# apache/bifromq

Measured on NVIDIA H100. Metric: publish-topics matched/sec @10M filters, higher is better.
Workload: dtype u8/u32 (byte and integer work)

## Files before the change

bifromq_b200/csrc/capi.cu:

```cuda
#include <cuda_runtime.h>

#include <algorithm>
#include <atomic>
#include <chrono>
#include <cstdio>
#include <cstdlib>
#include <cstring>
#include <memory>
#include <mutex>
#include <thread>
#include <string>
#include <vector>

#include "../../include/bfq_gpumatch.h"
#include "codec.h"
#include "cuda_buf.h"
#include "index_builder.h"
#include "fanout.h"
#include "lease.h"
#include "match_kernels.cuh"

using namespace bfq;

struct Snapshot {
    int device = 0;
    uint64_t generation = 0;
    DeviceBuf<Slot> d_slots, d_roots;
    DeviceBuf<uint32_t> d_segs, d_pfxP, d_pfxG;
    DeviceBuf<uint8_t> d_rkind, d_tags;
    FlatIndex flat;
    struct TenantHost {
        std::shared_ptr<const KVBlob> kv;
        std::shared_ptr<const std::vector<uint8_t>> rkind;
        std::shared_ptr<const TenantFan> fan;
    };
    struct FanTable {
        DeviceBuf<uint32_t> d_rdeliv, d_gmem_off, d_gmem_deliv;
        DeviceBuf<uint8_t> d_gordered;
        uint32_t n_deliverers = 0;
    };
    struct UrlTable {
        DeviceBuf<unsigned long long> d_words;
        DeviceBuf<long long> d_word;
        DeviceBuf<uint32_t> d_len;
        uint32_t member_bits = 1;
    };
    std::mutex fan_mu;
    std::shared_ptr<FanTable> fan;
    std::shared_ptr<UrlTable> urls;
    std::vector<TenantHost> th;
    uint64_t garbage_slots = 0;
    int64_t delta_commits = 0;
    size_t l2_window_bytes = 0;
    bool locate(int64_t rank, size_t* ti, int64_t* local) const {
        if (rank < 0 || rank >= flat.n_routes || flat.tenants.empty()) return false;
        size_t lo = 0, hi = flat.tenants.size();
        while (hi - lo > 1) {
            const size_t mid = (lo + hi) / 2;
            if (flat.tenants[mid].lo <= rank) lo = mid;
            else hi = mid;
        }
        *ti = lo;
        *local = rank - flat.tenants[lo].lo;
        return *local < flat.tenants[lo].n_routes;
    }
    int64_t device_bytes() const {
        return (int64_t) (d_slots.bytes() + d_tags.bytes() + d_roots.bytes() + d_segs.bytes() + d_rkind.bytes() + d_pfxP.bytes() + d_pfxG.bytes());
    }
    ~Snapshot() { cudaSetDevice(device); }
};

constexpr int MAX_CHUNKS = 8;

struct Workspace {
    int device = 0;
    cudaStream_t stream = nullptr, copy_stream = nullptr, work_stream[2] = {nullptr, nullptr};
    cudaEvent_t ev[2] = {nullptr, nullptr};
    cudaEvent_t ev_h2d[MAX_CHUNKS] = {};
    cudaEvent_t evk[2] = {nullptr, nullptr};
    cudaEvent_t ev_done = nullptr;
    std::vector<cudaEvent_t> ev_use;
    uint64_t tab_generation = ~0ull;
    std::vector<uint8_t> tab_blob;
    std::vector<int64_t> tab_off;
    std::vector<int32_t> tab_caps;
    int32_t tab_n = -1;
    bool any_cap = true;
    DeviceBuf<int32_t> d_tenant_tab;
    PinnedBuf<int32_t> h_tenant_tab;
    DeviceBuf<uint8_t> d_topics;
    DeviceBuf<int64_t> d_topic_off;
    DeviceBuf<int32_t> d_topic_tenant;
    DeviceBuf<uint32_t> d_span_begin, d_span_count, d_route_count, d_overflow, d_flagged, d_kept, d_defer;
    DeviceBuf<uint2> d_ranges, d_scratch, d_ranges_c;
    DeviceBuf<uint8_t> d_scan_tmp;
    DeviceBuf<uint32_t> d_cnt, d_new_begin, d_final_begin, d_final_count;
    DeviceBuf<uint32_t> d_ord_keys, d_leader, d_order;
    DeviceBuf<unsigned long long> d_hash_tab;
    DeviceBuf<uint32_t> d_hist;
    size_t hash_stride = 0, hist_stride = 0;
    DeviceBuf<uint3> d_throttled;
    DeviceBuf<unsigned long long> d_counters;
    PinnedBuf<unsigned long long> h_counters;
    DeviceBuf<unsigned long long> d_exp_counts;
    DeviceBuf<long long> d_bud_bytes;
    DeviceBuf<uint8_t> d_bud_bw, d_bud_flags;
    DeviceBuf<uint32_t> d_bud_dp, d_bud_list;
    DeviceBuf<unsigned long long> d_bud_ctr;
    DeviceBuf<uint32_t> d_fo_counts, d_fo_base, d_pack_topic, d_pack_rank, d_pack_member;
    DeviceBuf<long long> d_pack_offsets;
    DeviceBuf<uint8_t> d_fo_tmp;
    DeviceBuf<uint32_t> d_dl_topic_tmp, d_dl_pair_tmp, d_dl_pcount, d_package_tenant, d_dl_pack_topic, d_match_rank, d_match_member;
    DeviceBuf<unsigned long long> d_dl_totals;
    DeviceBuf<long long> d_package_off, d_dl_pack_off, d_match_off;
    DeviceBuf<uint8_t> d_dl_tmp;
    DeviceBuf<uint32_t> d_os_flag, d_os_u32, d_pack_pub;
    DeviceBuf<unsigned long long> d_os_items, d_os_check, d_os_key;
    DeviceBuf<long long> d_pack_pub_off;
    PinnedBuf<uint32_t> h_span_begin, h_span_count, h_route_count;
    PinnedBuf<uint2> h_ranges;
    PinnedBuf<uint3> h_throttled;

    cudaError_t init(int dev) {
        device = dev;
        cudaError_t e = cudaStreamCreateWithFlags(&stream, cudaStreamNonBlocking);
        if (e == cudaSuccess) e = cudaStreamCreateWithFlags(&copy_stream, cudaStreamNonBlocking);
        for (auto& w : work_stream)
            if (e == cudaSuccess) e = cudaStreamCreateWithFlags(&w, cudaStreamNonBlocking);
        for (auto& x : ev)
            if (e == cudaSuccess) e = cudaEventCreate(&x);
        for (auto& x : evk)
            if (e == cudaSuccess) e = cudaEventCreate(&x);
        for (auto& x : ev_h2d)
            if (e == cudaSuccess) e = cudaEventCreateWithFlags(&x, cudaEventDisableTiming);
        if (e == cudaSuccess) e = cudaEventCreateWithFlags(&ev_done, cudaEventDisableTiming);
        return e;
    }
    ~Workspace() {
        cudaSetDevice(device);
        for (auto& e : ev) if (e) cudaEventDestroy(e);
        for (auto& e : evk) if (e) cudaEventDestroy(e);
        for (auto& e : ev_h2d) if (e) cudaEventDestroy(e);
        if (ev_done) cudaEventDestroy(ev_done);
        for (auto& e : ev_use) cudaEventDestroy(e);
        if (copy_stream) cudaStreamDestroy(copy_stream);
        for (auto& w : work_stream) if (w) cudaStreamDestroy(w);
        if (stream) cudaStreamDestroy(stream);
    }
};

struct Pool {
    std::mutex mu;
    std::vector<Workspace*> idle;
    int device = 0;
    bool closed = false;
    ~Pool() {
        cudaSetDevice(device);
        for (Workspace* w : idle) delete w;
    }
};

struct bfq_result {
    bfq_index* owner = nullptr;
    std::shared_ptr<Pool> pool;
    std::shared_ptr<Snapshot> snap;
    Workspace* ws = nullptr;
    int64_t n_topics = 0, n_ranges = 0, n_throttled = 0;
    const uint32_t *span_begin = nullptr, *span_count = nullptr, *route_count = nullptr;
    const bfq_range* ranges = nullptr;
    const bfq_throttled* throttled = nullptr;
    double ms[4] = {0, 0, 0, 0};
};

struct bfq_index {
    int device = 0;
    std::mutex mu;
    std::mutex stage_mu;
    Staging staging;
    std::shared_ptr<Snapshot> snap;
    uint64_t next_generation = 1;
// ... 62 lines not shown
            pool->idle.push_back(w);
            return;
        }
    }
    cudaSetDevice(pool->device);
    delete w;
}

struct CoreOut {
    int64_t n_ranges = 0, n_throttled = 0, n_overflow = 0, n_flagged = 0, n_launches = 0, n_deferred = 0, n_leaders = 0;
    uint64_t want_dyn = 0, want_thr = 0;
    int64_t chunk_throttled[MAX_CHUNKS] = {};
};

int32_t resolve_tenants(Workspace* w, const Snapshot* s, const uint8_t* tenants, const int64_t* tenant_off, int32_t n_tenants,
                        const int32_t* max_p, const int32_t* max_g, cudaStream_t stream) {
    if (n_tenants < 0) return fail(BFQ_E_INVALID, "n_tenants < 0");
    if (n_tenants >= (1 << 30)) return fail(BFQ_E_RANGE, "more than 2^30 tenants in one batch");
    const size_t nt = (size_t) std::max(n_tenants, 1);
    const size_t blob_n = n_tenants ? (size_t) (tenant_off[n_tenants] - tenant_off[0]) : 0;
    bool same = w->tab_generation == s->generation && w->tab_n == n_tenants && w->tab_blob.size() == blob_n;
    if (same && n_tenants > 0) {
        same = memcmp(w->tab_blob.data(), tenants + tenant_off[0], blob_n) == 0;
        for (int32_t i = 0; same && i <= n_tenants; i++) same = w->tab_off[i] == tenant_off[i] - tenant_off[0];
        for (int32_t i = 0; same && i < n_tenants; i++)
            same = w->tab_caps[i] == (max_p ? max_p[i] : 0x7FFFFFFF) && w->tab_caps[nt + i] == (max_g ? max_g[i] : 0x7FFFFFFF);
    }
    if (same) return BFQ_OK;
    BFQ_CUDA_TRY(w->h_tenant_tab.reserve(3 * nt));
    BFQ_CUDA_TRY(w->d_tenant_tab.reserve(3 * nt));
    w->tab_blob.assign(tenants ? tenants + (n_tenants ? tenant_off[0] : 0) : nullptr, tenants ? tenants + (n_tenants ? tenant_off[0] : 0) + blob_n : nullptr);
    w->tab_off.resize(nt + 1);
    w->tab_caps.assign(2 * nt, 0x7FFFFFFF);
    bool any_cap = false;
    for (int32_t i = 0; i < n_tenants; i++) {
        std::string t((const char*) tenants + tenant_off[i], (size_t) (tenant_off[i + 1] - tenant_off[i]));
        auto it = s->flat.tenant_ordinal.find(t);
        const int32_t mp = max_p ? max_p[i] : 0x7FFFFFFF, mg = max_g ? max_g[i] : 0x7FFFFFFF;
        w->h_tenant_tab.p[i] = it == s->flat.tenant_ordinal.end() ? -1 : (int32_t) it->second;
        w->h_tenant_tab.p[nt + i] = mp;
        w->h_tenant_tab.p[2 * nt + i] = mg;
        w->tab_off[i] = tenant_off[i] - tenant_off[0];
        w->tab_caps[i] = mp;
        w->tab_caps[nt + i] = mg;
        any_cap = any_cap || mp != 0x7FFFFFFF || mg != 0x7FFFFFFF;
    }
    if (n_tenants > 0) w->tab_off[n_tenants] = tenant_off[n_tenants] - tenant_off[0];
    BFQ_CUDA_TRY(cudaMemcpyAsync(w->d_tenant_tab.p, w->h_tenant_tab.p, 3 * nt * sizeof(int32_t), cudaMemcpyHostToDevice, stream));
    w->tab_generation = s->generation;
    w->tab_n = n_tenants;
    w->any_cap = any_cap;
    return BFQ_OK;
}

struct SubBatch {
    int64_t begin = 0, n = 0, n_total = 0;
    int chunk = 0;
    uint64_t dyn_off = 0, dyn_cap = 0;
    uint64_t thr_off = 0, thr_cap = 0;
};
constexpr int32_t BFQ_RETRY_GROW = -100;

int32_t prepare_workspace(bfq_index* h, Workspace* w, int64_t n, int n_chunks, int32_t n_tenants) {
    const size_t nn = (size_t) std::max<int64_t>(n, 1);
    if (n >= (int64_t) 0x3FFFFFFF) return fail(BFQ_E_INVALID, "too many topics in one batch");
    BFQ_CUDA_TRY(w->d_span_begin.reserve(nn));
    BFQ_CUDA_TRY(w->d_span_count.reserve(nn));
    BFQ_CUDA_TRY(w->d_route_count.reserve(nn));
    BFQ_CUDA_TRY(w->d_overflow.reserve(nn));
    BFQ_CUDA_TRY(w->d_flagged.reserve(nn));
    BFQ_CUDA_TRY(w->d_kept.reserve(nn));
    BFQ_CUDA_TRY(w->d_defer.reserve(nn));
    BFQ_CUDA_TRY(w->d_counters.reserve(CTR_COUNT * MAX_CHUNKS));
    BFQ_CUDA_TRY(w->h_counters.reserve(CTR_COUNT * MAX_CHUNKS));
    const uint64_t dyn_base = (uint64_t) n * INLINE_RANGES;
    if (dyn_base >= 0xF0000000ull) return fail(BFQ_E_RANGE, "batch too large for 32-bit range indices; split the batch");
    const size_t min_dyn = std::max<size_t>((size_t) n_chunks << 18, nn);
    if (w->d_ranges.cap < dyn_base + min_dyn) BFQ_CUDA_TRY(w->d_ranges.reserve((size_t) (dyn_base + std::max<size_t>(1 << 20, min_dyn))));
    const int64_t per_chunk = (n + n_chunks - 1) / n_chunks + 1;
    if (per_chunk >= h->order_min) {
        BFQ_CUDA_TRY(w->d_ord_keys.reserve(nn));
        BFQ_CUDA_TRY(w->d_leader.reserve(nn));
        BFQ_CUDA_TRY(w->d_order.reserve(nn));
        const size_t hist_stride = order_scratch_words(per_chunk, n_tenants);
        const size_t hash_stride = order_hash_entries(per_chunk);
        if (hist_stride > w->hist_stride) {
            BFQ_CUDA_TRY(w->d_hist.reserve(2 * hist_stride));
            w->hist_stride = hist_stride;
        }
        if (hash_stride > w->hash_stride) {
            BFQ_CUDA_TRY(w->d_hash_tab.reserve(2 * hash_stride));
            w->hash_stride = hash_stride;
        }
    }
    if (w->d_throttled.cap < ((size_t) n_chunks << 14)) BFQ_CUDA_TRY(w->d_throttled.reserve(std::max<size_t>(1 << 16, (size_t) n_chunks << 14)));
    return BFQ_OK;
}

SubBatch whole_batch(Workspace* w, int64_t n) {
    SubBatch sb;
    sb.begin = 0;
    sb.n = sb.n_total = n;
    sb.dyn_cap = w->d_ranges.cap - (uint64_t) n * INLINE_RANGES;
    sb.thr_cap = w->d_throttled.cap;
    return sb;
}

struct CoreCtx {
    bfq_index* h;
    Workspace* w;
    const Snapshot* s;
    const uint8_t* d_topics;
    const int64_t* d_topic_off;
    const int32_t* d_topic_tenant;
    int32_t n_tenants;
    cudaStream_t stream;
};

MatchParams core_params(const CoreCtx& c, const SubBatch& sb) {
    Workspace* w = c.w;
    const size_t nt = (size_t) std::max(c.n_tenants, 1);
    const int64_t b = sb.begin;
    MatchParams p{};
    p.slots = c.s->d_slots.p;
    p.roots = c.s->d_roots.p;
    p.tags = reinterpret_cast<const uint4*>(c.s->d_tags.p);
    p.n_blocks = c.s->flat.n_blocks;
    p.topics = c.d_topics;
    p.topic_off = c.d_topic_off + b;
    p.topic_tenant = c.d_topic_tenant + b;
    p.tenant_root = w->d_tenant_tab.p;
    p.max_pfanout = w->d_tenant_tab.p + nt;
    p.max_gfanout = w->d_tenant_tab.p + 2 * nt;
    p.n_tenants = c.n_tenants;
    p.n_topics = sb.n;
    p.span_begin = w->d_span_begin.p + b;
    p.span_count = w->d_span_count.p + b;
    p.route_count = w->d_route_count.p + b;
    p.overflow_list = w->d_overflow.p + b;
    p.defer_list = w->d_defer.p + b;
    p.flagged_list = w->d_flagged.p + b;
    p.counters = w->d_counters.p + (size_t) sb.chunk * CTR_COUNT;
    p.ranges = w->d_ranges.p + (uint64_t) b * INLINE_RANGES;
    p.dyn_base = (uint64_t) (sb.n_total - b) * INLINE_RANGES + sb.dyn_off;
    p.ranges_cap = p.dyn_base + sb.dyn_cap;
    p.max_ctas_per_sm = c.h->tier0_ctas_per_sm;
    return p;
}

CapsParams caps_params(const CoreCtx& c, const SubBatch& sb, const MatchParams& p) {
    CapsParams q{};
    q.flagged_list = p.flagged_list;
    q.topic_tenant = p.topic_tenant;
    q.max_pfanout = p.max_pfanout;
    q.max_gfanout = p.max_gfanout;
    q.span_begin = p.span_begin;
    q.span_count = p.span_count;
    q.ranges = p.ranges;
    q.segs = c.s->d_segs.p;
    q.rkind = c.s->d_rkind.p;
    q.pfx_persistent = c.s->d_pfxP.p;
    q.pfx_group = c.s->d_pfxG.p;
    q.kept_count = c.w->d_kept.p + sb.begin;
    q.counters = p.counters;
    q.throttled = c.w->d_throttled.p + sb.thr_off;
    q.throttled_cap = sb.thr_cap;
    q.topic_base = (uint32_t) sb.begin;
    return q;
}

bool wants_order(const CoreCtx& c, const SubBatch& sb) {
    return sb.n >= c.h->order_min && c.w->d_order.cap >= (size_t) (sb.begin + sb.n) && c.w->hist_stride > 0 &&
           c.w->hist_stride >= order_scratch_words(sb.n, c.n_tenants) && c.w->hash_stride >= order_hash_entries(sb.n);
}

int32_t enqueue_core(const CoreCtx& c, const SubBatch& sb, CoreOut* out) {
    Workspace* w = c.w;
    cudaStream_t stream = c.stream;
    const int64_t n = sb.n, b = sb.begin;
    MatchParams p = core_params(c, sb);
    if (c.s->l2_window_bytes > 0) {
        cudaStreamAttrValue attr{};
        attr.accessPolicyWindow.base_ptr = c.s->d_tags.p;
        attr.accessPolicyWindow.num_bytes = c.s->l2_window_bytes;
        attr.accessPolicyWindow.hitRatio = 1.0f;
        attr.accessPolicyWindow.hitProp = cudaAccessPropertyPersisting;
        attr.accessPolicyWindow.missProp = cudaAccessPropertyStreaming;
        cudaStreamSetAttribute(stream, cudaStreamAttributeAccessPolicyWindow, &attr);
        cudaGetLastError();
    }
    BFQ_CUDA_TRY(cudaMemsetAsync(p.counters, 0, CTR_COUNT * sizeof(unsigned long long), stream));
    bool ordered = false, dedup = false;
    if (wants_order(c, sb)) {
        const int slot = sb.chunk & 1;
        OrderParams q{};
        q.n_topics = n;
        q.topics = c.d_topics;
        q.topic_off = p.topic_off;
        q.topic_tenant = p.topic_tenant;
        q.n_tenants = c.n_tenants;
        q.keys = w->d_ord_keys.p + b;
        q.leader = w->d_leader.p + b;
        q.order = w->d_order.p + b;
        q.hash_tab = w->d_hash_tab.p + (size_t) slot * w->hash_stride;
        q.hash_mask = order_hash_entries(n) - 1;
        q.hist = w->d_hist.p + (size_t) slot * w->hist_stride;
        q.dedup = c.h->dedup ? 1 : 0;
        q.dedup_hash_mask = c.h->dedup_hash_bits >= 64 ? ~0ull : (1ull << c.h->dedup_hash_bits) - 1;
        q.counters = p.counters;
        BFQ_CUDA_TRY(launch_order(q, stream));
        p.order = q.order;
        p.order_count = p.counters + CTR_NLEAD;
        out->n_launches += 3;
        ordered = true;
        dedup = q.dedup != 0;
    }
    if (n > 0) {
        if (sb.chunk == 0) BFQ_CUDA_TRY(cudaEventRecord(w->evk[0], stream));
        launch_match_lanes(p, stream);
        if (sb.chunk == 0) BFQ_CUDA_TRY(cudaEventRecord(w->evk[1], stream));
        p.work_list = p.defer_list;
        p.n_work = -1;
        launch_match(p, false, 0, stream);
        out->n_launches += 2;
        if (ordered && dedup) {
            FinalizeParams f{};
            f.n_topics = n;
            f.leader = w->d_leader.p + b;
            f.span_begin = p.span_begin;
            f.span_count = p.span_count;
            f.route_count = p.route_count;
            f.flagged_list = p.flagged_list;
            f.counters = p.counters;
            f.second_pass = 0;
            launch_finalize(f, stream);
            out->n_launches += 1;
        }
        if (w->any_cap) {
            CapsParams q = caps_params(c, sb, p);
            q.n_flagged = -1;
            launch_caps(q, stream);
            out->n_launches += 2;
        }
    }
    BFQ_CUDA_TRY(cudaGetLastError());
    return BFQ_OK;
}

int32_t copy_counters(const CoreCtx& c, const SubBatch& sb) {
    BFQ_CUDA_TRY(cudaMemcpyAsync(c.w->h_counters.p + (size_t) sb.chunk * CTR_COUNT, c.w->d_counters.p + (size_t) sb.chunk * CTR_COUNT,
                             CTR_COUNT * sizeof(unsigned long long), cudaMemcpyDeviceToHost, c.stream));
    return BFQ_OK;
}

int32_t finish_core(const CoreCtx& c, const SubBatch& sb, CoreOut* out, bool* reran, cudaEvent_t done = nullptr) {
    Workspace* w = c.w;
    cudaStream_t stream = c.stream;
    unsigned long long* hc = w->h_counters.p + (size_t) sb.chunk * CTR_COUNT;
    if (reran) *reran = false;
    if (done) BFQ_CUDA_TRY(cudaEventSynchronize(done));
    else BFQ_CUDA_TRY(cudaStreamSynchronize(stream));
    out->n_overflow += (int64_t) hc[CTR_OVERFLOW];
    out->n_deferred += (int64_t) hc[CTR_DEFER];
    if (hc[CTR_OVERFLOW] > 0) {
        MatchParams p = core_params(c, sb);
        const uint64_t capF = (uint64_t) c.s->flat.max_nodes_per_depth + 2;
        const uint64_t capR = 2 * ((uint64_t) c.s->flat.max_tenant_nodes + 2) + 2;
        const uint64_t per_warp = 4 * capF + capR;
        uint64_t warps = std::min<uint64_t>(hc[CTR_OVERFLOW], std::max<uint64_t>(8, (1ull << 31) / (per_warp * sizeof(uint2))));
        warps = std::min<uint64_t>(warps, (uint64_t) device_sm_count() * 8);
        warps = (warps + 7) / 8 * 8;
        if (w->d_scratch.cap < (size_t) (warps * per_warp)) {
            BFQ_CUDA_TRY(cudaDeviceSynchronize());
            BFQ_CUDA_TRY(w->d_scratch.reserve((size_t) (warps * per_warp)));
        }
        p.scratch = w->d_scratch.p;
        p.scratch_frontier_cap = capF;
        p.scratch_ranges_cap = capR;
        p.work_list = p.overflow_list;
        p.n_work = (int64_t) hc[CTR_OVERFLOW];
        launch_match(p, true, (int) warps, stream);
        out->n_launches++;
        if (w->hist_stride > 0 && c.h->dedup && wants_order(c, sb)) {
            FinalizeParams f{};
            f.n_topics = sb.n;
            f.leader = w->d_leader.p + sb.begin;
            f.span_begin = p.span_begin;
            f.span_count = p.span_count;
            f.route_count = p.route_count;
            f.flagged_list = p.flagged_list;
            f.counters = p.counters;
            f.second_pass = 1;
            launch_finalize(f, stream);
            out->n_launches++;
        }
        if (w->any_cap) {
            CapsParams q = caps_params(c, sb, p);
            q.n_flagged = -1;
            launch_caps(q, stream);
            out->n_launches += 2;
        }
        BFQ_CUDA_TRY(cudaGetLastError());
        int32_t rc = copy_counters(c, sb);
        if (rc != BFQ_OK) return rc;
        BFQ_CUDA_TRY(cudaStreamSynchronize(stream));
        if (hc[CTR_ERROR] != 0) return fail(BFQ_E_STATE, "tier-2 scratch exhausted (index statistics inconsistent)");
        if (reran) *reran = true;
    }
    if (hc[CTR_RANGES] > sb.dyn_cap) {
        out->want_dyn = std::max<uint64_t>(out->want_dyn, hc[CTR_RANGES]);
        return BFQ_RETRY_GROW;
// ... 1830 lines not shown
```

bifromq_b200/csrc/match_kernels.cu:

```cuda
#include "match_kernels.cuh"
#include "hash_probe.cuh"

#include <cub/device/device_scan.cuh>

#include <algorithm>
#include <mutex>
#include <cstdlib>

namespace bfq {

namespace {

constexpr int WARPS_PER_CTA = 8;
constexpr int STAGE_BYTES = 256;
constexpr uint32_t FR_CAP = 64;
constexpr uint32_t RG_CAP = 48;
constexpr uint32_t NONE31 = 0x7FFFFFFFu;
constexpr unsigned FULL = 0xFFFFFFFFu;

struct WarpSmem {
    uint8_t stage[STAGE_BYTES];
    uint32_t keyw[8];
    uint4 fr[2][FR_CAP];
    uint2 rg[RG_CAP];
// ... 169 lines not shown
        return;
    }
    const int maxP = p.max_pfanout[tenant], maxG = p.max_gfanout[tenant];
    const bool flag_p = maxP != 0x7FFFFFFF && acc_p > (uint64_t) (maxP < 0 ? 0 : maxP);
    const bool flag_g = maxG != 0x7FFFFFFF && acc_g > (uint64_t) (maxG < 0 ? 0 : maxG);
    const bool flagged = flag_p || flag_g;
    unsigned long long base = 0;
    if (n_rg > 0) {
        if (lane == 0) base = atomicAdd(&p.counters[CTR_RANGES], (unsigned long long) n_rg);
        base = __shfl_sync(FULL, base, 0);
        base += p.dyn_base;
        if (base + n_rg <= p.ranges_cap)
            for (uint32_t i = lane; i < n_rg; i += 32) p.ranges[base + i] = rg[i];
    }
    if (lane == 0) {
        p.span_begin[t] = (uint32_t) base;
        p.span_count[t] = n_rg | (flagged ? SPAN_FLAGGED : 0u);
        p.route_count[t] = acc_r;
        if (flagged) {
            const unsigned long long idx = atomicAdd(&p.counters[CTR_FLAGGED], 1ull);
            p.flagged_list[idx] = t;
        }
    }
}

template <bool kBig>
__global__ void __launch_bounds__(WARPS_PER_CTA * 32) match_topics_kernel(const MatchParams p) {
    __shared__ WarpSmem sm[WARPS_PER_CTA];
    const int lane = threadIdx.x & 31, wid = threadIdx.x >> 5;
    WarpSmem& ws = sm[wid];
    const int64_t gw = (int64_t) blockIdx.x * WARPS_PER_CTA + wid;
    const int64_t nw = (int64_t) gridDim.x * WARPS_PER_CTA;
    if (kBig) {
        uint2* basep = p.scratch + (uint64_t) gw * (4 * p.scratch_frontier_cap + p.scratch_ranges_cap);
        uint4* fr_a = reinterpret_cast<uint4*>(basep);
        uint4* fr_b = reinterpret_cast<uint4*>(basep + 2 * p.scratch_frontier_cap);
        uint2* rg = basep + 4 * p.scratch_frontier_cap;
        const uint32_t capF = (uint32_t) min((uint64_t) 0x3FFFFFFFull, p.scratch_frontier_cap);
        const uint32_t capR = (uint32_t) min((uint64_t) SPAN_COUNT_MASK, p.scratch_ranges_cap);
        for (int64_t it = gw; it < p.n_work; it += nw) match_one<true>(p, ws, p.work_list[it], lane, fr_a, fr_b, rg, capF, capR);
    } else if (p.work_list) {
        const int64_t n_work = p.n_work >= 0 ? p.n_work : (int64_t) p.counters[CTR_DEFER];
        for (int64_t it = gw; it < n_work; it += nw)
            match_one<false>(p, ws, p.work_list[it], lane, ws.fr[0], ws.fr[1], ws.rg, FR_CAP, RG_CAP);
    } else {
        for (int64_t it = gw; it < p.n_topics; it += nw)
            match_one<false>(p, ws, (uint32_t) it, lane, ws.fr[0], ws.fr[1], ws.rg, FR_CAP, RG_CAP);
    }
}


constexpr int L_WARPS = 4;
constexpr int64_t LARGE_BATCH_TOPICS = 1 << 17;
constexpr int LARGE_BATCH_CTAS_PER_SM = 4;
constexpr int L_MAXLV = 12;
constexpr int L_CHUNK = 32;
constexpr int TENANT_CAPPED = 1 << 30;

struct LaneSmem {
    uint16_t lv[L_MAXLV + 1][32];
    uint2 stk[L_MAXLV + 1][32];
    uint32_t stkm[L_MAXLV + 1][32];
    int64_t m_off[L_CHUNK];
    uint32_t m_t[L_CHUNK];
    uint32_t m_len[L_CHUNK];
    int32_t m_tenant[L_CHUNK];
    int32_t m_root[L_CHUNK];
    uint32_t c_root[8];
    int32_t c_ord;
};

template <bool kRootStep, bool kPrefetch, bool kNA>
__global__ void __launch_bounds__(L_WARPS * 32) match_topics_lane_kernel(const MatchParams p) {
    __shared__ LaneSmem sm[L_WARPS];
    const int lane = threadIdx.x & 31, wid = threadIdx.x >> 5;
    LaneSmem& ws = sm[wid];
    const uint32_t lt_mask = (1u << lane) - 1;
    const int64_t n = (p.order && p.order_count) ? (int64_t) *p.order_count : p.n_topics;

    int64_t next = 0, end = 0, cstart = 0;
    bool exhausted = false;
    bool have = false, bad = false;
    uint32_t t = 0, node = 0 , plusf = NONE31, meta = 0, pending = 0, n_rg = 0, acc_r = 0;
    uint32_t acc_p = 0, acc_g = 0;
    uint2* rg_out = nullptr;
    int64_t my_off = 0;
    int len = 0, level = 0, tenant = 0;

    auto emit = [&](uint32_t first, uint32_t count, bool multi, uint32_t caps) {
        if (n_rg >= INLINE_RANGES) {
            if (n_rg == INLINE_RANGES) {
                const unsigned long long at = p.dyn_base + atomicAdd(&p.counters[CTR_RANGES], (unsigned long long) SPILL_RANGES);
                if (at + SPILL_RANGES <= p.ranges_cap) {
                    uint2* dst = p.ranges + at;
                    const uint2* src = rg_out - INLINE_RANGES;
#pragma unroll
                    for (int j = 0; j < (int) INLINE_RANGES; j++) dst[j] = src[j];
                    rg_out = dst + INLINE_RANGES;
                } else {
                    bad = true;
                }
            } else if (n_rg >= SPILL_RANGES) {
                bad = true;
            }
        }
        if (!bad) *rg_out++ = make_uint2(first, multi ? (count | RANGE_MULTI) : count);
        n_rg++;
        acc_r += count;
        const uint32_t cp = caps & 0xFFu, cg = (caps >> 8) & 0xFFu;
        acc_p = (acc_p + cp) | (cp == 0xFFu ? 0x80000000u : 0u);
        acc_g = (acc_g + cg) | (cg == 0xFFu ? 0x80000000u : 0u);
    };
    auto finish = [&]() {
        if (bad) {
            const unsigned long long idx = atomicAdd(&p.counters[CTR_DEFER], 1ull);
            p.defer_list[idx] = t;
            p.span_begin[t] = 0;
            p.span_count[t] = SPAN_OVERFLOW;
            p.route_count[t] = 0;
        } else {
            bool flagged = false;
            if ((tenant & TENANT_CAPPED) && (acc_p | acc_g)) {
                const int tn = tenant & ~TENANT_CAPPED;
                const int maxP = p.max_pfanout[tn], maxG = p.max_gfanout[tn];
                const bool flag_p = maxP != 0x7FFFFFFF && acc_p > (uint32_t) (maxP < 0 ? 0 : maxP);
                const bool flag_g = maxG != 0x7FFFFFFF && acc_g > (uint32_t) (maxG < 0 ? 0 : maxG);
                flagged = flag_p || flag_g;
            }
            p.span_begin[t] = (uint32_t) ((rg_out - n_rg) - p.ranges);
            p.span_count[t] = n_rg | (flagged ? SPAN_FLAGGED : 0u);
            p.route_count[t] = acc_r;
            if (flagged) {
                const unsigned long long idx = atomicAdd(&p.counters[CTR_FLAGGED], 1ull);
                p.flagged_list[idx] = t;
            }
        }
        have = false;
    };

    while (true) {
        const unsigned idle = __ballot_sync(FULL, !have);
        if (idle) {
            if (next >= end && !exhausted) {
                unsigned long long c = 0;
                if (lane == 0) c = atomicAdd(&p.counters[CTR_CHUNK], (unsigned long long) L_CHUNK);
                c = __shfl_sync(FULL, c, 0);
                if ((int64_t) c >= n) {
                    exhausted = true;
                } else {
                    cstart = next = (int64_t) c;
                    end = min(n, next + L_CHUNK);
                    __syncwarp();
                    for (int i = lane; i < (int) (end - cstart); i += 32) {
                        const uint32_t ti = p.order ? p.order[cstart + i] : (uint32_t) (cstart + i);
                        const int64_t o = p.topic_off[ti], o2 = p.topic_off[ti + 1];
                        int tn = p.topic_tenant[ti];
                        const bool tn_ok = tn >= 0 && tn < p.n_tenants;
                        if (!tn_ok) tn = 0;
                        if (kPrefetch) {
                            if (((o + 28) >> 7) != (o >> 7)) asm volatile("prefetch.global.L2 [%0];" ::"l"(p.topics + o + 28));
                        }
                        const bool sys = o2 > o && p.topics[o] == '$';
                        const bool capped = p.max_pfanout[tn] != 0x7FFFFFFF || p.max_gfanout[tn] != 0x7FFFFFFF;
                        ws.m_t[i] = ti;
                        ws.m_off[i] = o;
                        ws.m_len[i] = (uint32_t) min((int64_t) 0x7FFFFFFF, o2 - o) | (sys ? 0x80000000u : 0u);
                        ws.m_tenant[i] = tn | (capped ? TENANT_CAPPED : 0);
                        const int ro = tn_ok ? p.tenant_root[tn] : -1;
                        ws.m_root[i] = ro;
                        if (i == 0) {
                            ws.c_ord = ro;
                            if (ro >= 0) {
                                uint32_t rw[16];
                                load_payload(p.roots + ro, rw);
#pragma unroll
                                for (int j = 0; j < 8; j++) ws.c_root[j] = rw[8 + j];
                            }
                        }
                    }
                    __syncwarp();
                }
            }
            if (next < end) {
                const int64_t idx = next + __popc(idle & lt_mask);
                const bool take = !have && idx < end;
                next = min(end, next + (int64_t) __popc(idle));
                if (take) {
                    const int i = (int) (idx - cstart);
                    t = ws.m_t[i];
                    my_off = ws.m_off[i];
                    const uint32_t lenw = ws.m_len[i];
                    len = (int) (lenw & 0x7FFFFFFFu);
                    tenant = ws.m_tenant[i];
                    const int root_ord = ws.m_root[i];
                    n_rg = 0; acc_r = 0; acc_p = 0; acc_g = 0; pending = 0;
                    rg_out = p.ranges + (uint64_t) idx * INLINE_RANGES;
                    bad = len > 65535;
                    have = true;
                    ws.lv[0][lane] = 0;
                    level = -1;
                    node = (uint32_t) root_ord;
                    plusf = NONE31;
                    if (root_ord < 0 || bad) {
                        finish();
                    } else if (!kRootStep) {
                        uint32_t rw[16];
                        if (root_ord == ws.c_ord) {
#pragma unroll
                            for (int j = 0; j < 8; j++) rw[8 + j] = ws.c_root[j];
                        } else {
                            load_payload(p.roots + root_ord, rw);
                        }
                        const bool sys = lenw >> 31;
                        if (!sys && rw[W_HASH_COUNT] > 0) emit(rw[W_HASH_FIRST], rw[W_HASH_COUNT], rw[W_META] & FLAG_HASH_MULTI, (rw[W_CAPS] >> 16));
                        const uint32_t rplus = (sys || rw[W_PLUS] == NONE) ? NONE31 : rw[W_PLUS];
                        const uint32_t has_exact = rw[W_META] & FLAG_HAS_EXACT;
                        if ((has_exact || rplus != NONE31) && !bad) {
                            node = child_ref(ROOT_BASE + (uint32_t) root_ord, rw);
                            plusf = rplus;
                            meta = rw[W_META];
                            level = 0;
                        } else {
                            finish();
                        }
                    }
                }
            } else if (idle == FULL) {
                break;
            }
        }
        if (have) {
            const bool rootstep = kRootStep && level < 0;
            const int lvl = rootstep ? 0 : level;
            const int s = ws.lv[lvl][lane];
            const int rem = len - s;
            const uint64_t a = (uint64_t) (uintptr_t) p.topics + (uint64_t) my_off + (uint64_t) s;
            const uint4* qp = reinterpret_cast<const uint4*>(a & ~15ull);
            const int o = (int) (a & 15);
            const int need = o + min(rem, 28);
            uint4 q0 = make_uint4(0u, 0u, 0u, 0u), q1 = q0, q2 = q0;
            if (need > 0) q0 = __ldg(qp);
            if (need > 16) q1 = __ldg(qp + 1);
            if (need > 32) q2 = __ldg(qp + 2);
            const uint32_t plus = plusf;
            const bool has_plus = rootstep || plus != NONE31;
            uint32_t pw[16];
            if (has_plus) {
                if (rootstep) load_payload<false>(p.roots + node, pw);
                else load_payload<kNA>(p.slots + plus, pw);
            }
            uint32_t k[7];
            {
                const uint32_t X[12] = {q0.x, q0.y, q0.z, q0.w, q1.x, q1.y, q1.z, q1.w, q2.x, q2.y, q2.z, q2.w};
                const bool by2 = o & 8, by1 = o & 4;
                uint32_t Y[10], Z[8];
#pragma unroll
                for (int j = 0; j < 10; j++) Y[j] = by2 ? X[j + 2] : X[j];
#pragma unroll
                for (int j = 0; j < 8; j++) Z[j] = by1 ? Y[j + 1] : Y[j];
                const int sh = (o & 3) * 8;
#pragma unroll
                for (int j = 0; j < 7; j++) k[j] = __funnelshift_r(Z[j], Z[j + 1], sh);
            }
            const uint32_t first_byte = k[0] & 0xFFu;
            int q = 28;
#pragma unroll
            for (int j = 6; j >= 0; j--) {
                const uint32_t y = k[j] ^ 0x2F2F2F2Fu;
                const uint32_t hz = (y - 0x01010101u) & ~y & 0x80808080u;
                if (hz) q = 4 * j + ((__ffs(hz) - 1) >> 3);
            }
            const int tlen = min(q, rem);
            const bool last = tlen == rem;
            if (rootstep) {
                const bool sys = len > 0 && first_byte == '$';
                if (!sys && pw[W_HASH_COUNT] > 0) emit(pw[W_HASH_FIRST], pw[W_HASH_COUNT], pw[W_META] & FLAG_HASH_MULTI, (pw[W_CAPS] >> 16));
                const uint32_t rplus = (sys || pw[W_PLUS] == NONE) ? NONE31 : pw[W_PLUS];
                const uint32_t has_exact = pw[W_META] & FLAG_HAS_EXACT;
                if ((has_exact || rplus != NONE31) && !bad) {
// ... 214 lines not shown
    const int len = min(hlen, 4 * ORDER_WINDOW_WORDS);
    const int rest = key_bits - tenant_bits;
    const int b0 = rest / 3 + (rest % 3 > 0), b1 = rest / 3 + (rest % 3 > 1), b2 = rest / 3;
    uint32_t run = 0x9E3779B1u, dig[3] = {0u, 0u, 0u};
    int lvl = 0;
#pragma unroll
    for (int j = 0; j < ORDER_WINDOW_WORDS; j++) {
        uint32_t m = 4 * j < len ? match_bytes(k[j], 0x2F2F2F2Fu) : 0u;
        while (m && lvl < 3) {
            const int byte = (__ffs(m) - 1) >> 3;
            m &= m - 1;
            if (((k[j] >> (8 * byte)) & 0xFFu) != 0x2Fu) continue;
            const uint32_t part = byte ? (k[j] & (0xFFFFFFFFu >> (32 - 8 * byte))) : 0u;
            const uint32_t hh = (run ^ part) * 0x85EBCA77u + (uint32_t) (4 * j + byte);
            dig[lvl++] = (hh ^ (hh >> 15)) * 0x9E3779B1u;
        }
        run = (run ^ k[j]) * 0xCC9E2D51u;
        run ^= run >> 13;
    }
    const int closed = lvl;
    if (lvl < 3) dig[lvl] = ((run + (uint32_t) len) ^ (run >> 15)) * 0x9E3779B1u;
    uint32_t key = tenant_bits ? ((uint32_t) max(tn, 0) & ((1u << tenant_bits) - 1u)) : 0u;
    key = (key << b0) | (b0 ? dig[0] >> (32 - b0) : 0u);
    key = (key << b1) | (b1 && closed >= 1 ? dig[1] >> (32 - b1) : 0u);
    key = (key << b2) | (b2 && closed >= 2 ? dig[2] >> (32 - b2) : 0u);
    const uint32_t bucket = key_bits > q.hist_bits ? key >> (key_bits - q.hist_bits) : key;
    q.keys[i] = bucket;
    atomicAdd(&q.hist[bucket], 1u);
}

constexpr int SCAN_THREADS = 1024, SCAN_PER_BLOCK = 4096;
__device__ __forceinline__ uint32_t block_exclusive_scan(uint32_t v, uint32_t* warp_sums, uint32_t& total) {
    const int lane = threadIdx.x & 31, wid = threadIdx.x >> 5;
    uint32_t inc = v;
#pragma unroll
    for (int o = 1; o < 32; o <<= 1) {
        const uint32_t y = __shfl_up_sync(FULL, inc, o);
        if (lane >= o) inc += y;
    }
    if (lane == 31) warp_sums[wid] = inc;
    __syncthreads();
    if (wid == 0) {
        const uint32_t ws = warp_sums[lane];
        uint32_t winc = ws;
#pragma unroll
        for (int o = 1; o < 32; o <<= 1) {
            const uint32_t y = __shfl_up_sync(FULL, winc, o);
            if (lane >= o) winc += y;
        }
        warp_sums[lane] = winc - ws;
        if (lane == 31) warp_sums[32] = winc;
    }
    __syncthreads();
    total = warp_sums[32];
    const uint32_t r = warp_sums[wid] + inc - v;
    __syncthreads();
    return r;
}
__global__ void __launch_bounds__(SCAN_THREADS) order_scan_kernel(const OrderKernelParams q) {
    __shared__ uint32_t warp_sums[33];
    __shared__ bool is_last;
    uint4* hv = reinterpret_cast<uint4*>(q.hist + (size_t) blockIdx.x * SCAN_PER_BLOCK) + threadIdx.x;
    const uint4 c = *hv;
    uint32_t total;
    const uint32_t ex = block_exclusive_scan(c.x + c.y + c.z + c.w, warp_sums, total);
    *hv = make_uint4(ex, ex + c.x, ex + c.x + c.y, ex + c.x + c.y + c.z);
    if (threadIdx.x == 0) {
        q.blk_tot[blockIdx.x] = total;
        __threadfence();
        is_last = atomicAdd(q.ticket, 1u) == gridDim.x - 1;
    }
    __syncthreads();
    if (!is_last) return;
    __threadfence();
    const uint32_t v = threadIdx.x < gridDim.x ? *((volatile uint32_t*) q.blk_tot + threadIdx.x) : 0u;
    const uint32_t pfx = block_exclusive_scan(v, warp_sums, total);
    if (threadIdx.x < gridDim.x) q.blk_pfx[threadIdx.x] = pfx;
    if (threadIdx.x == 0) q.counters[CTR_NLEAD] = total;
}
__global__ void __launch_bounds__(256) order_scatter_kernel(const OrderKernelParams q) {
    const int64_t i = (int64_t) blockIdx.x * blockDim.x + threadIdx.x;
    if (i >= q.n_topics || q.leader[i] != (uint32_t) i) return;
    const uint32_t b = q.keys[i];
    q.order[q.blk_pfx[b / SCAN_PER_BLOCK] + atomicAdd(&q.hist[b], 1u)] = (uint32_t) i;
}

__global__ void __launch_bounds__(256) finalize_kernel(const FinalizeParams p) {
    const int64_t i = (int64_t) blockIdx.x * blockDim.x + threadIdx.x;
    if (i >= p.n_topics) return;
    const uint32_t l = p.leader[i];
    if (l == (uint32_t) i) return;
    if (p.second_pass && p.span_count[i] != SPAN_OVERFLOW) return;
    const uint32_t sc = p.span_count[l];
    p.span_begin[i] = p.span_begin[l];
    p.span_count[i] = sc;
    p.route_count[i] = p.route_count[l];
    if (sc & SPAN_FLAGGED) p.flagged_list[atomicAdd(&p.counters[CTR_FLAGGED], 1ull)] = (uint32_t) i;
}

__global__ void compact_counts_kernel(const CompactParams p) {
    const int64_t i = (int64_t) blockIdx.x * blockDim.x + threadIdx.x;
    if (i < p.n_topics) p.counts[i] = (p.leader && p.leader[i] != (uint32_t) i) ? 0u : (p.span_count[i] & SPAN_COUNT_MASK);
}
__global__ void compact_total_kernel(const CompactParams p) {
    *p.total_out = (unsigned long long) p.new_begin[p.n_topics - 1] + p.counts[p.n_topics - 1];
}
__global__ void compact_gather_kernel(const CompactParams p) {
    const int64_t i = (int64_t) blockIdx.x * blockDim.x + threadIdx.x;
    if (i >= p.n_topics) return;
    const uint32_t l = p.leader ? p.leader[i] : (uint32_t) i;
    const uint32_t c = p.span_count[i] & SPAN_COUNT_MASK;
    const uint32_t nb = p.new_begin[l];
    if (l == (uint32_t) i) {
        const uint32_t ob = p.span_begin[i];
        if ((uint64_t) nb + c <= p.ranges_out_cap)
            for (uint32_t j = 0; j < c; j++) p.ranges_out[nb + j] = p.ranges[ob + j];
    }
    p.final_begin[i] = nb + p.out_base;
    p.final_count[i] = c;
}

constexpr int CAPS_THREADS = 128;

struct SegIter {
    const uint2* ranges;
    const uint32_t* segs;
    uint32_t n;
    template <typename F>
    __device__ __forceinline__ void for_range(uint32_t j, F&& f) const {
        const uint2 r = ranges[j];
        if (r.y & RANGE_MULTI) {
            const uint32_t nseg = segs[2 * (uint64_t) r.x];
            for (uint32_t s = 0; s < nseg; s++) f(segs[2 * ((uint64_t) r.x + 1 + s)], segs[2 * ((uint64_t) r.x + 1 + s) + 1]);
        } else {
            f(r.x, r.y);
        }
    }
};

__device__ __forceinline__ void caps_one(const CapsParams& p, uint32_t t);
__global__ void __launch_bounds__(CAPS_THREADS) caps_kernel(const CapsParams p) {
    if (p.n_flagged >= 0) {
        caps_one(p, p.flagged_list[blockIdx.x]);
        return;
    }
    const unsigned long long b = p.counters[CTR_FLAGGED2], e = p.counters[CTR_FLAGGED];
    for (unsigned long long j = b + blockIdx.x; j < e; j += gridDim.x) {
        caps_one(p, p.flagged_list[j]);
        __syncthreads();
    }
}
__device__ __forceinline__ void caps_one(const CapsParams& p, uint32_t t) {
    const int tenant = p.topic_tenant[t];
    const uint64_t maxP = (uint64_t) max(p.max_pfanout[tenant], 0), maxG = (uint64_t) max(p.max_gfanout[tenant], 0);
    SegIter it{p.ranges + p.span_begin[t], p.segs, p.span_count[t] & SPAN_COUNT_MASK};
    __shared__ unsigned long long kept;
    if (threadIdx.x == 0) kept = 0;
    __syncthreads();
    unsigned long long my_kept = 0;
    for (uint32_t j = threadIdx.x; j < it.n; j += CAPS_THREADS) {
        it.for_range(j, [&](uint32_t first, uint32_t count) {
            uint64_t baseP = 0, baseG = 0;
            for (uint32_t q = 0; q < it.n; q++)
                it.for_range(q, [&](uint32_t f2, uint32_t c2) {
                    if (f2 < first) {
                        baseP += p.pfx_persistent[f2 + c2] - p.pfx_persistent[f2];
                        baseG += p.pfx_group[f2 + c2] - p.pfx_group[f2];
                    }
                });
            const uint64_t cntP = p.pfx_persistent[first + count] - p.pfx_persistent[first];
            const uint64_t cntG = p.pfx_group[first + count] - p.pfx_group[first];
            if (baseP + cntP <= maxP && baseG + cntG <= maxG) {
                my_kept += count;
// ... 430 lines not shown
```

bifromq_b200/csrc/match_kernels.cuh:

```cuda
#pragma once
#include <cuda_runtime.h>
#include <stdint.h>

#include "trie_layout.h"

namespace bfq {

enum : int {
    CTR_RANGES = 0,
    CTR_OVERFLOW = 1,
    CTR_FLAGGED = 2,
    CTR_THROTTLED = 3,
    CTR_ROUTES = 4,
    CTR_ERROR = 5,
    CTR_DEFER = 6,
    CTR_CHUNK = 7,
    CTR_NLEAD = 8,
    CTR_FLAGGED2 = 9,
    CTR_COUNT = 12,
};

constexpr uint32_t SPAN_FLAGGED = 0x80000000u;
constexpr uint32_t SPAN_OVERFLOW = 0x40000000u;
constexpr uint32_t SPAN_COUNT_MASK = 0x3FFFFFFFu;

struct MatchParams {
    const Slot* slots;
    const uint4* tags;
    const Slot* roots;
    uint32_t n_blocks;
    const uint8_t* topics;
    const int64_t* topic_off;
    const int32_t* topic_tenant;
    const int32_t* tenant_root;
    const int32_t* max_pfanout;
    const int32_t* max_gfanout;
    int32_t n_tenants;
    int64_t n_topics;
    const uint32_t* order;
    const unsigned long long* order_count;
    int32_t max_ctas_per_sm;
    const uint32_t* work_list;
    int64_t n_work;
    uint32_t* span_begin;
    uint32_t* span_count;
    uint32_t* route_count;
    uint2* ranges;
    uint64_t ranges_cap;
    uint64_t dyn_base;
    uint32_t* overflow_list;
    uint32_t* defer_list;
    uint32_t* flagged_list;
    unsigned long long* counters;
    uint2* scratch;
    uint64_t scratch_frontier_cap;
    uint64_t scratch_ranges_cap;
};

struct CapsParams {
    const uint32_t* flagged_list;
    int64_t n_flagged;
    const int32_t* topic_tenant;
    const int32_t* max_pfanout;
    const int32_t* max_gfanout;
    const uint32_t* span_begin;
    const uint32_t* span_count;
    const uint2* ranges;
    const uint32_t* segs;
    const uint8_t* rkind;
    const uint32_t* pfx_persistent;
    const uint32_t* pfx_group;
    uint3* throttled;
    uint32_t topic_base;
    uint64_t throttled_cap;
    uint32_t* kept_count;
    unsigned long long* counters;
};

struct ExpandParams {
    int64_t n_topics;
    const uint32_t* span_begin;
    const uint32_t* span_count;
    const uint32_t* route_count;
    const uint32_t* kept_count;
    const uint2* ranges;
    const uint32_t* segs;
    unsigned long long* counts;
    int64_t* offsets;
    int64_t* ranks;
    int64_t rank_cap;
    const uint32_t* flagged_list;
    int64_t n_flagged;
    const int32_t* topic_tenant;
    const int32_t* max_pfanout;
    const int32_t* max_gfanout;
    const uint8_t* rkind;
    const uint32_t* pfx_persistent;
    const uint32_t* pfx_group;
};
cudaError_t launch_expand(const ExpandParams& p, void* d_scan_tmp, size_t* tmp_bytes, cudaStream_t stream, int phase);

enum : uint8_t {
    BUDGET_BYTES_THROTTLED = 1,
    BUDGET_NO_PERSISTENT_BW = 2,
    BUDGET_NO_TRANSIENT_BW = 4,
    BUDGET_METERED = 8,
    BUDGET_DROPS = 7,
};
enum : int {
    BUD_LISTED = 0,
    BUD_BAD_SIZE = 1,
    BUD_DROP_BYTES = 2,
    BUD_DROP_PBW = 3,
    BUD_DROP_TBW = 4,
    BUD_CTR_COUNT = 8,
};
struct BudgetParams {
    ExpandParams e;
    int32_t n_tenants;
    const int32_t* msg_bytes;
    const long long* max_bytes;
    const uint8_t* bandwidth;
    uint32_t* delivered_p;
    uint8_t* flags;
    uint32_t* list;
    int64_t n_listed;
    unsigned long long* ctr;
};
cudaError_t launch_budget(const BudgetParams& q, void* d_scan_tmp, size_t* tmp_bytes, cudaStream_t stream, int phase);

struct OrderParams {
    int64_t n_topics;
    const uint8_t* topics;
    const int64_t* topic_off;
    const int32_t* topic_tenant;
    int32_t n_tenants;
    uint32_t* keys;
    uint32_t* leader;
    uint32_t* order;
    unsigned long long* hash_tab;
    uint32_t hash_mask;
    uint32_t* hist;
    int dedup;
    uint64_t dedup_hash_mask;
    unsigned long long* counters;
};
size_t order_scratch_words(int64_t n_topics, int32_t n_tenants);
uint32_t order_hash_entries(int64_t n_topics);
cudaError_t launch_order(const OrderParams& q, cudaStream_t stream);

struct FinalizeParams {
    int64_t n_topics;
    const uint32_t* leader;
    uint32_t* span_begin;
    uint32_t* span_count;
    uint32_t* route_count;
    uint32_t* flagged_list;
    unsigned long long* counters;
    int second_pass;
};
void launch_finalize(const FinalizeParams& p, cudaStream_t stream);

void launch_match_lanes(const MatchParams& p, cudaStream_t stream);
void launch_match(const MatchParams& p, bool tier2, int n_warps_tier2, cudaStream_t stream);
void launch_caps(const CapsParams& p, cudaStream_t stream);

constexpr uint32_t INLINE_RANGES = 12;
constexpr uint32_t SPILL_RANGES = 64;

struct CompactParams {
    int64_t n_topics;
    const uint32_t* span_begin;
    const uint32_t* span_count;
    const uint2* ranges;
    const uint32_t* leader;
    uint32_t* counts;
    uint32_t* new_begin;
    uint32_t* final_begin;
    uint32_t* final_count;
    uint2* ranges_out;
    uint64_t ranges_out_cap;
    uint32_t out_base;
    unsigned long long* total_out;
};
cudaError_t launch_compact(const CompactParams& p, void* d_scan_tmp, size_t* tmp_bytes, cudaStream_t stream, int phase);
int match_kernel_smem_bytes();
int device_sm_count();

struct RankShiftRegion {
    uint64_t base, len;
    int32_t delta;
};
void launch_rank_shift(Slot* slots, const RankShiftRegion* d_regions, int n_regions, cudaStream_t stream);
struct RankShiftSlot {
    uint32_t slot;
    int32_t delta;
};
void launch_rank_shift_listed(Slot* slots, const RankShiftSlot* d_list, int64_t n, cudaStream_t stream);
void launch_scatter_records(Slot* slots, const uint32_t* d_ids, const Slot* d_recs, int64_t n, cudaStream_t stream);
struct RankRun {
    uint32_t new_lo, len;
    uint32_t src_lo;
    uint32_t packed;
    uint32_t dP, dG;
};
struct AssembleRankParams {
    uint8_t* rkind;
    uint32_t *pfxP, *pfxG;
    const uint8_t* old_rkind;
    const uint32_t *old_pfxP, *old_pfxG;
    const uint8_t* up_rkind;
    const uint32_t *up_pfxP, *up_pfxG;
    const RankRun* runs;
    int32_t n_runs;
    int64_t n;
    uint32_t tailP, tailG;
};
void launch_assemble_rank_arrays(const AssembleRankParams& p, cudaStream_t stream);

}
```

Baseline: 1.134 billion.

## Write match span results to position-ordered 16-byte records, scatter in finalize

In the ordered path, the match kernel now writes each topic's span begin/count/route count as one 16-byte record indexed by its sorted position rather than three scattered per-topic stores. The order scatter kernel records each leader's position in the keys array, and finalize always runs in ordered mode to gather records back into per-topic arrays and propagate them to duplicates. The aim is coalesced stores from the match kernel. In exchange there is an extra buffer, an always-on finalize pass and an indirect gather. Deferred topics still fall through to the old leader-copy logic.

Measured after the change: 1.270 billion (median of 6 runs). 1.12x the previous value.

```diff
diff --git a/bifromq_b200/csrc/capi.cu b/bifromq_b200/csrc/capi.cu
--- a/bifromq_b200/csrc/capi.cu
+++ b/bifromq_b200/csrc/capi.cu
@@ -96,6 +96,7 @@
     DeviceBuf<uint8_t> d_scan_tmp;
     DeviceBuf<uint32_t> d_cnt, d_new_begin, d_final_begin, d_final_count;
     DeviceBuf<uint32_t> d_ord_keys, d_leader, d_order;
+    DeviceBuf<SpanRecord> d_pos_rec;
     DeviceBuf<unsigned long long> d_hash_tab;
     DeviceBuf<uint32_t> d_hist;
     size_t hash_stride = 0, hist_stride = 0;
@@ -324,6 +325,7 @@
         BFQ_CUDA_TRY(w->d_ord_keys.reserve(nn));
         BFQ_CUDA_TRY(w->d_leader.reserve(nn));
         BFQ_CUDA_TRY(w->d_order.reserve(nn));
+        BFQ_CUDA_TRY(w->d_pos_rec.reserve(nn));
         const size_t hist_stride = order_scratch_words(per_chunk, n_tenants);
         const size_t hash_stride = order_hash_entries(per_chunk);
         if (hist_stride > w->hist_stride) {
@@ -412,7 +414,8 @@
 }
 
 bool wants_order(const CoreCtx& c, const SubBatch& sb) {
-    return sb.n >= c.h->order_min && c.w->d_order.cap >= (size_t) (sb.begin + sb.n) && c.w->hist_stride > 0 &&
+    return sb.n >= c.h->order_min && c.w->d_order.cap >= (size_t) (sb.begin + sb.n) &&
+           c.w->d_pos_rec.cap >= (size_t) (sb.begin + sb.n) && c.w->hist_stride > 0 &&
            c.w->hist_stride >= order_scratch_words(sb.n, c.n_tenants) && c.w->hash_stride >= order_hash_entries(sb.n);
 }
 
@@ -432,7 +435,7 @@
         cudaGetLastError();
     }
     BFQ_CUDA_TRY(cudaMemsetAsync(p.counters, 0, CTR_COUNT * sizeof(unsigned long long), stream));
-    bool ordered = false, dedup = false;
+    bool ordered = false;
     if (wants_order(c, sb)) {
         const int slot = sb.chunk & 1;
         OrderParams q{};
@@ -453,9 +456,9 @@
         BFQ_CUDA_TRY(launch_order(q, stream));
         p.order = q.order;
         p.order_count = p.counters + CTR_NLEAD;
+        p.pos_rec = w->d_pos_rec.p + b;
         out->n_launches += 3;
         ordered = true;
-        dedup = q.dedup != 0;
     }
     if (n > 0) {
         if (sb.chunk == 0) BFQ_CUDA_TRY(cudaEventRecord(w->evk[0], stream));
@@ -465,10 +468,12 @@
         p.n_work = -1;
         launch_match(p, false, 0, stream);
         out->n_launches += 2;
-        if (ordered && dedup) {
+        if (ordered) {
             FinalizeParams f{};
             f.n_topics = n;
             f.leader = w->d_leader.p + b;
+            f.pos = w->d_ord_keys.p + b;
+            f.pos_rec = p.pos_rec;
             f.span_begin = p.span_begin;
             f.span_count = p.span_count;
             f.route_count = p.route_count;
diff --git a/bifromq_b200/csrc/match_kernels.cu b/bifromq_b200/csrc/match_kernels.cu
--- a/bifromq_b200/csrc/match_kernels.cu
+++ b/bifromq_b200/csrc/match_kernels.cu
@@ -275,6 +275,7 @@
     bool exhausted = false;
     bool have = false, bad = false;
     uint32_t t = 0, node = 0 , plusf = NONE31, meta = 0, pending = 0, n_rg = 0, acc_r = 0;
+    uint32_t pos = 0;
     uint32_t acc_p = 0, acc_g = 0;
     uint2* rg_out = nullptr;
     int64_t my_off = 0;
@@ -304,13 +305,20 @@
         acc_p = (acc_p + cp) | (cp == 0xFFu ? 0x80000000u : 0u);
         acc_g = (acc_g + cg) | (cg == 0xFFu ? 0x80000000u : 0u);
     };
+    auto put_span = [&](uint32_t begin, uint32_t count, uint32_t routes, uint32_t deferred) {
+        if (p.order) {
+            p.pos_rec[pos] = SpanRecord{begin, count, routes, deferred};
+        } else {
+            p.span_begin[t] = begin;
+            p.span_count[t] = count;
+            p.route_count[t] = routes;
+        }
+    };
     auto finish = [&]() {
         if (bad) {
             const unsigned long long idx = atomicAdd(&p.counters[CTR_DEFER], 1ull);
             p.defer_list[idx] = t;
-            p.span_begin[t] = 0;
-            p.span_count[t] = SPAN_OVERFLOW;
-            p.route_count[t] = 0;
+            put_span(0u, SPAN_OVERFLOW, 0u, 1u);
         } else {
             bool flagged = false;
             if ((tenant & TENANT_CAPPED) && (acc_p | acc_g)) {
@@ -320,9 +328,8 @@
                 const bool flag_g = maxG != 0x7FFFFFFF && acc_g > (uint32_t) (maxG < 0 ? 0 : maxG);
                 flagged = flag_p || flag_g;
             }
-            p.span_begin[t] = (uint32_t) ((rg_out - n_rg) - p.ranges);
-            p.span_count[t] = n_rg | (flagged ? SPAN_FLAGGED : 0u);
-            p.route_count[t] = acc_r;
+            put_span((uint32_t) ((rg_out - n_rg) - p.ranges),
+                     n_rg | (flagged ? SPAN_FLAGGED : 0u), acc_r, 0u);
             if (flagged) {
                 const unsigned long long idx = atomicAdd(&p.counters[CTR_FLAGGED], 1ull);
                 p.flagged_list[idx] = t;
@@ -388,6 +395,7 @@
                     const int root_ord = ws.m_root[i];
                     n_rg = 0; acc_r = 0; acc_p = 0; acc_g = 0; pending = 0;
                     rg_out = p.ranges + (uint64_t) idx * INLINE_RANGES;
+                    pos = (uint32_t) idx;
                     bad = len > 65535;
                     have = true;
                     ws.lv[0][lane] = 0;
@@ -768,13 +776,25 @@
     const int64_t i = (int64_t) blockIdx.x * blockDim.x + threadIdx.x;
     if (i >= q.n_topics || q.leader[i] != (uint32_t) i) return;
     const uint32_t b = q.keys[i];
-    q.order[q.blk_pfx[b / SCAN_PER_BLOCK] + atomicAdd(&q.hist[b], 1u)] = (uint32_t) i;
+    const uint32_t at = q.blk_pfx[b / SCAN_PER_BLOCK] + atomicAdd(&q.hist[b], 1u);
+    q.order[at] = (uint32_t) i;
+    q.keys[i] = at;
 }
 
 __global__ void __launch_bounds__(256) finalize_kernel(const FinalizeParams p) {
     const int64_t i = (int64_t) blockIdx.x * blockDim.x + threadIdx.x;
     if (i >= p.n_topics) return;
     const uint32_t l = p.leader[i];
+    if (!p.second_pass) {
+        const SpanRecord r = p.pos_rec[p.pos[l]];
+        if (!r.deferred) {
+            p.span_begin[i] = r.span_begin;
+            p.span_count[i] = r.span_count;
+            p.route_count[i] = r.route_count;
+            if (l != (uint32_t) i && (r.span_count & SPAN_FLAGGED)) p.flagged_list[atomicAdd(&p.counters[CTR_FLAGGED], 1ull)] = (uint32_t) i;
+            return;
+        }
+    }
     if (l == (uint32_t) i) return;
     if (p.second_pass && p.span_count[i] != SPAN_OVERFLOW) return;
     const uint32_t sc = p.span_count[l];
diff --git a/bifromq_b200/csrc/match_kernels.cuh b/bifromq_b200/csrc/match_kernels.cuh
--- a/bifromq_b200/csrc/match_kernels.cuh
+++ b/bifromq_b200/csrc/match_kernels.cuh
@@ -24,6 +24,14 @@
 constexpr uint32_t SPAN_OVERFLOW = 0x40000000u;
 constexpr uint32_t SPAN_COUNT_MASK = 0x3FFFFFFFu;
 
+struct __align__(16) SpanRecord {
+    uint32_t span_begin;
+    uint32_t span_count;
+    uint32_t route_count;
+    uint32_t deferred;
+};
+static_assert(sizeof(SpanRecord) == 16, "a span record is one 16-byte store");
+
 struct MatchParams {
     const Slot* slots;
     const uint4* tags;
@@ -39,6 +47,7 @@
     int64_t n_topics;
     const uint32_t* order;
     const unsigned long long* order_count;
+    SpanRecord* pos_rec;
     int32_t max_ctas_per_sm;
     const uint32_t* work_list;
     int64_t n_work;
@@ -152,6 +161,8 @@
 struct FinalizeParams {
     int64_t n_topics;
     const uint32_t* leader;
+    const uint32_t* pos;
+    const SpanRecord* pos_rec;
     uint32_t* span_begin;
     uint32_t* span_count;
     uint32_t* route_count;
```
